# JaworWr/CUDA-ray-tracer

Hardware: AMD Instinct MI355X
Metric: Mrays/sec, 20spheres.yml @1920x1080 (higher is better)
Workload: dtype f64

## Files before the change

cuda-ray-tracer_amd/csrc/rt_capi.cpp:

```cpp
#include <hip/hip_runtime.h>

#include <algorithm>
#include <cmath>
#include <cstdarg>
#include <cstdio>
#include <cstdlib>
#include <cstring>
#include <memory>
#include <new>
#include <string>
#include <vector>

#include "mi355rt.h"
#include "rt_launch.h"
#include "rt_scene_dev.h"
#include "rt_scene_image.hpp"
#include "rt_frame_host.hpp"
#include "rt_set_scene.h"
#include "scene-exception.h"
#include "scene.h"
#include "camera.h"

#define RT_KERNELS(V)                                                                                                                              \
    {RT_CAT(rt_launch_trace, V), RT_CAT(rt_launch_wavefront, V),  RT_CAT(rt_launch_ray_list, V),      RT_CAT(rt_launch_gbuffer, V),   RT_CAT(rt_launch_pick, V), \
// ... 170 lines not shown
    bool zero_counters = false;
    DevMem<uint64_t> d_stamps;
    DevMem<double> d_camx, d_camy;
    size_t n_stamp_rows = 0;
    uint64_t frame = 0;
    uint32_t tag = 0;
    DevMem<uint32_t> d_order, d_tiles;
    MappedWords h_listed;
    uint32_t ord_split = 0;
    std::vector<double> cub_coefs;
    bool lean_ok = false;
    bool lean_now = true;
    uint32_t wg_slots = 1536;
    int lean_force = 0;
    bool ord_on = true;
    Staging pick;
    Staging ext;
    Staging rq;
    Scratch pth;
    DevMem<SetSceneStatus> d_ss_status;
    DevMem<unsigned char> d_ss_stage;
};

#ifdef RT_DIAGNOSTIC_BUILD
extern "C" int rt_abi_version(void) { return RT_ABI_VERSION | RT_ABI_DIAGNOSTIC; }
#else
extern "C" int rt_abi_version(void) { return RT_ABI_VERSION; }
#endif

extern "C" const char *rt_last_error(void) { return g_last_error.c_str(); }
// ... 222 lines not shown
    fa.height = rh;
    fa.max_refl = sd->max_reflections;
    fa.rank = cfg.rank;
    fa.world = cfg.world;
    fa.band_rows = kf * cfg.band_rows;
    fa.local_rows = kf * ctx->local_rows;
    fa.tiles_x = (rw + RT_TILE - 1) / RT_TILE;
    fa.n_tiles = fa.tiles_x * ((fa.local_rows + RT_TILE - 1) / RT_TILE);
    fa.rgba8 = (ctx->ssaa == 1u && cfg.format == RT_FMT_RGBA8) ? 1u : 0u;
    fa.ord_plain = (cfg.flags & RT_FLAG_PLAIN_ORDER) ? 1u : 0u;
    ctx->ord_split = (cfg.flags & RT_FLAG_NOSPLIT) ? 0u : RT_ORD_SPLIT_CLASSES;
    if (const char *e = std::getenv("MI355RT_SPLIT_CLASSES")) ctx->ord_split = (uint32_t) std::atoi(e) & 15u;
    int cus = 0;
    if (hipDeviceGetAttribute(&cus, hipDeviceAttributeMultiprocessorCount, device) == hipSuccess && cus > 0) ctx->wg_slots = 6u * (uint32_t) cus;
    if (const char *e = std::getenv("MI355RT_LEAN")) ctx->lean_force = (e[0] == 'a') ? 1 : ((e[0] == 'n') ? -1 : 0);
}

static int create_scene(rt_ctx *ctx, const rt_scene_desc *sd, rtp::SceneImage &im)
{
    FrameArgs &fa = ctx->fa;
    im = rtp::scene_image(*sd, ctx->cfg.flags, fa);
    ctx->cub_coefs = im.cub_coefs;
    ctx->lean_ok = im.lean_ok && !std::getenv("MI355RT_NOLEAN");
    if (!(ctx->cfg.flags & RT_FLAG_SIMPLE)) {
        const size_t lds = rt_wavefront_lds_bytes_strict(fa.stage_bytes, sd->n_lights, (int) fa.has_mirror, fa.cull ? fa.n_us : 0u, 0, fa.n_cub);
        if (lds > 160u * 1024u) return fail(RT_ERR_SCENE, "rt_create: scene needs %zu bytes of LDS per workgroup (limit 160 KiB)", lds);
    }
    if (ctx->adaptive && (size_t) sd->n_objects * (sizeof(DevObject) + sizeof(UsEntry)) > 160u * 1024u)
        return fail(RT_ERR_SCENE, "rt_create: adaptive supersampling stages %zu bytes of LDS per workgroup (limit 160 KiB)",
                    (size_t) sd->n_objects * (sizeof(DevObject) + sizeof(UsEntry)));
// ... 67 lines not shown
    return device_table(ctx->d_geo_xy, xy.data(), sizeof(uint32_t) * 2u * hpx, "halo coordinates");
}

static int create_order_state(rt_ctx *ctx)
{
    FrameArgs &fa = ctx->fa;
    const uint32_t flags = ctx->cfg.flags;
    if (!(flags & (RT_FLAG_SIMPLE | RT_FLAG_STATIC_ORDER)) && fa.n_tiles > 0 && fa.n_tiles <= RT_ORD_MAX_TILES) {
        fa.ord_stride = (RT_ORD_HDR + 17u * fa.n_tiles + 15u) & ~15u;
        if (int rc = device_table(ctx->d_order, nullptr, sizeof(uint32_t) * (3u * (size_t) fa.ord_stride + fa.n_tiles), "order")) return rc;
        fa.order_state = ctx->d_order;
        if (hipHostMalloc((void **) &ctx->h_listed.p, 64, hipHostMallocMapped | hipHostMallocPortable) == hipSuccess) {
            ctx->h_listed[0] = 0;
            ctx->h_listed[1] = 0;
            ctx->h_listed[2] = 0xFFFFFFFFu;
            if (hipHostGetDevicePointer((void **) &fa.ord_host, ctx->h_listed, 0) != hipSuccess) {
                ctx->h_listed.reset();
                fa.ord_host = nullptr;
            }
        } else {
            ctx->h_listed.p = nullptr;
            (void) hipGetLastError();
        }
    }
    if (!(flags & RT_FLAG_SIMPLE) && fa.all_cullable && fa.n_tiles > 0) {
        if (int rc = device_table(ctx->d_tiles, nullptr, sizeof(uint32_t) * fa.n_tiles, "tile state")) return rc;
        fa.tile_state = ctx->d_tiles;
    }
    ctx->zero_counters = std::getenv("MI355RT_DEBUG_COUNTERS") != nullptr;
    if (ctx->zero_counters) {
// ... 99 lines not shown
}

static int timer_end(rt_ctx *ctx, hipStream_t stream, float *ms)
{
    if (!ms) return RT_OK;
    RT_HIP(hipEventRecord(ctx->ev1, stream));
    RT_HIP(hipEventSynchronize(ctx->ev1));
    RT_HIP(hipEventElapsedTime(ms, ctx->ev0, ctx->ev1));
    return RT_OK;
}

static void choose_schedule(rt_ctx *ctx, FrameArgs &fa)
{
    if (ctx->lean_ok && ctx->h_listed && ctx->lean_force == 0) {
        const uint32_t tiles = ((volatile uint32_t *) ctx->h_listed.p)[2];
        if (ctx->lean_now ? (uint64_t) tiles * 100u < (uint64_t) ctx->wg_slots * 62u : (uint64_t) tiles * 100u >= (uint64_t) ctx->wg_slots * 66u) ctx->lean_now = !ctx->lean_now;
    } else {
        ctx->lean_now = ctx->lean_force >= 0;
    }
    static const bool debug_order = std::getenv("MI355RT_DEBUG_ORDER") != nullptr;
    if (debug_order && ctx->h_listed)
        std::fprintf(stderr, "mi355rt: frame %llu: tiles with hits %u, list slots wanted %u, census %u, schedule %s\n", (unsigned long long) ctx->frame, ((volatile uint32_t *) ctx->h_listed.p)[2],
                     ((volatile uint32_t *) ctx->h_listed.p)[0], ((volatile uint32_t *) ctx->h_listed.p)[1], ctx->lean_now ? "lean" : "general");
    fa.lean = (ctx->lean_ok && ctx->lean_now && !fa.sparse) ? 1u : 0u;
}

static int rotate_launch_order(rt_ctx *ctx, FrameArgs &fa, hipStream_t stream)
{
    fa.ord_read = (uint32_t) (ctx->frame % 3u);
    fa.ord_write = (uint32_t) ((ctx->frame + 1u) % 3u);
    fa.ord_zero = (uint32_t) ((ctx->frame + 2u) % 3u);
    uint32_t cap = fa.n_tiles;
    if (ctx->h_listed) {
        const uint32_t seen = ((volatile uint32_t *) ctx->h_listed.p)[0], census = ((volatile uint32_t *) ctx->h_listed.p)[1];
        const uint64_t want = (uint64_t) seen + seen / 4u + 64u;
        if (want < cap) cap = (uint32_t) want;
        const uint64_t with_hits = (uint64_t) census * 16u;
        const uint64_t slots = ctx->wg_slots ? ctx->wg_slots : 1536u;
        const bool too_many = ctx->ord_on ? with_hits * 3u >= slots * 16u : with_hits >= slots * 4u;
        const bool too_dense = ctx->ord_on ? with_hits * 4u >= fa.n_tiles : with_hits * 5u >= fa.n_tiles;
        ctx->ord_on = !(too_many || too_dense);
    }
    fa.ord_cap = cap;
    fa.ord_on = ctx->ord_on ? 1u : 0u;
    fa.ord_split = (fa.sparse || fa.lean) ? 0u : ctx->ord_split;
    fa.ord_frame = (uint32_t) (ctx->frame % 0xFFFFFFF0ull) + 1u;
    if (fa.ord_frame == 1u && ctx->frame != 0u)
        RT_HIP(hipMemsetAsync(fa.order_state + 3u * (size_t) fa.ord_stride, 0, sizeof(uint32_t) * fa.n_tiles, stream));
    ctx->frame++;
    return RT_OK;
}

static int render_impl(rt_ctx *ctx, const double cam[16], void *dev_fb, void *stream_, float *ms, bool sparse, uint32_t sparse_cap)
{
    hipStream_t stream = (hipStream_t) stream_;
    FrameArgs &fa = ctx->fa;
    const bool ss = ctx->ssaa > 1u && !ctx->adaptive;
// ... 450 lines not shown
    a.coefs = dev->coefs;
    a.reflection = dev->reflection;
    a.albedo = dev->albedo;
    a.light_p = dev->light_p;
    a.light_color = dev->light_color;
    a.n_obj = fa.n_obj;
    a.n_lights = fa.n_lights;
    a.n_us = fa.n_us;
    a.n_gq = fa.n_gq;
    a.n_lin = fa.n_lin;
    a.off_us = fa.off_us;
    a.off_gq = fa.off_gq;
    a.off_lin = fa.off_lin;
    a.off_mat = fa.off_mat;
    a.has_mirror = fa.has_mirror;
    const hipError_t e = rt_launch_set_scene(&a, stream);
    if (e != hipSuccess) return fail(RT_ERR_DEVICE, "%s: kernel launch failed: %s", who, hipGetErrorString(e));
    return order_end(ctx, stream, capturing);
}

extern "C" int rt_set_scene(rt_ctx *ctx, const rt_scene_update *dev, void *stream)
{
    if (!ctx || !dev) return fail(RT_ERR_INVALID, "rt_set_scene: null argument");
    if (int rc = set_scene_check("rt_set_scene", ctx, dev)) return rc;
    return set_scene_enqueue("rt_set_scene", ctx, dev, (hipStream_t) stream);
}

extern "C" int rt_set_scene_host(rt_ctx *ctx, const rt_scene_update *host, void *stream_)
{
    if (!ctx || !host) return fail(RT_ERR_INVALID, "rt_set_scene_host: null argument");
// ... 251 lines not shown
```

cuda-ray-tracer_amd/csrc/rt_frame_host.hpp:

```cpp
#ifndef RT_FRAME_HOST_HPP
#define RT_FRAME_HOST_HPP

#include <algorithm>
#include <cmath>
#include <cstring>
#include <vector>

#include "rt_math.hpp"
#include "rt_scene_dev.h"

namespace rtf {

inline void camera_tables(uint32_t nx, uint32_t ny, double aspect, double tan_half_fov, std::vector<double> &cx, std::vector<double> &cy)
{
    cx.resize(nx);
    cy.resize(ny);
    for (uint32_t x = 0; x < nx; x++) {
        const double ndc_x = ((int) x + 0.5) / (int) nx;
        cx[x] = (2.0 * ndc_x - 1.0) * aspect * tan_half_fov;
    }
    for (uint32_t y = 0; y < ny; y++) {
        const double ndc_y = ((int) y + 0.5) / (int) ny;
        cy[y] = (2.0 * ndc_y - 1.0) * tan_half_fov;
    }
// ... 30 lines not shown
    }
    fa.cx_a = 2.0 * fa.aspect * fa.tan_half_fov / (double) fa.width;
    fa.cx_b = (1.0 / (double) fa.width - 1.0) * fa.aspect * fa.tan_half_fov;
    fa.cy_a = 2.0 * fa.tan_half_fov / (double) fa.height;
    fa.cy_b = (1.0 / (double) fa.height - 1.0) * fa.tan_half_fov;
    if (!(fa.cx_a > 0.0) || !(fa.cy_a > 0.0) || !std::isfinite(fa.cx_a) || !std::isfinite(fa.cy_a)) fa.tile_planes_ok = 0;
}

inline int64_t halo_global_row(uint32_t h, uint32_t band_rows, uint32_t world, uint32_t rank, uint32_t local_rows)
{
    const uint32_t b = h >> 1, rows = std::min(band_rows, local_rows - b * band_rows);
    const int64_t g0 = ((int64_t) b * world + rank) * band_rows;
    return (h & 1u) ? g0 + rows : g0 - 1;
}

}

#endif
```

cuda-ray-tracer_amd/csrc/rt_scene_dev.h:

```cpp
#ifndef RT_SCENE_DEV_H
#define RT_SCENE_DEV_H

#include <stddef.h>
#include <stdint.h>

enum {
    K_X3 = 0, K_Y3, K_Z3, K_X2Y, K_XY2, K_X2Z, K_XZ2, K_Y2Z, K_YZ2, K_XYZ,
    K_X2, K_Y2, K_Z2, K_XY, K_XZ, K_YZ,
    K_X, K_Y, K_Z, K_C
};

#define RT_CLS_CUBIC 1u
#define RT_CLS_SQUARE 2u
#define RT_CLS_CROSS 4u
#define RT_CLS_UNITSQ 8u

struct alignas(16) DevObject {
    double c[20];
    float albedo[3];
    float refl;
    uint32_t cls;
    uint32_t pad[3];
    double bs_center[3];
    double bs_radius;
// ... 77 lines not shown
    uint32_t *ord_host;
    uint32_t ord_stride, ord_read, ord_write, ord_zero;
    uint32_t ord_cap;
    uint32_t ord_on;
    uint32_t ord_plain;
    uint32_t ord_frame;
    uint32_t ord_split;
    uint32_t *tile_state;
    uint32_t frame_tag;
    uint32_t n_scan;
    uint32_t lean;
    double cub_rec[4][10];
    double cub_abs[4][4];
    uint32_t lights_plain;
    uint32_t pt_mask[2];
};

#define RT_CUB_AT_MAX 4
#define RT_CUB_REC 10
static_assert(offsetof(FrameArgs, cub_abs) == offsetof(FrameArgs, cub_rec) + sizeof(double) * 4 * RT_CUB_REC, "cub_abs directly behind cub_rec");
#define RT_TILE 16
#define RT_SCAN_TILES 64
#define RT_PAINT_TILES 16
#define RT_ORD_SPLIT_CLASSES 8u
#define RT_ORD_HDR 32
#define RT_ORD_MAX_TILES 262144u

#endif
```

cuda-ray-tracer_amd/csrc/rt_wavefront.hip:

```cpp
#include <hip/hip_runtime.h>
#include <cstdlib>

#include "rt_launch.h"
#include "rt_math.hpp"
#include "rt_scene_dev.h"
#include "rt_wavefront_math.hpp"

#ifndef RT_VARIANT
#error "define RT_VARIANT=strict|fast"
#endif

namespace RT_SYM(rtw) {

using namespace rtm;

#define RT_LOAD_LIGHTK(lk, l) \
    LightK lk; \
    lk.p[0] = clight[l].p[0]; lk.p[1] = clight[l].p[1]; lk.p[2] = clight[l].p[2]; \
    lk.sdir[0] = clight[l].sdir[0]; lk.sdir[1] = clight[l].sdir[1]; lk.sdir[2] = clight[l].sdir[2]; \
    lk.u2 = clight[l].u2; lk.inv_uu = clight[l].inv_uu; lk.len_u = clight[l].len_u; lk.four_u2 = clight[l].four_u2; \
    lk.s_yz = clight[l].s_yz; lk.s_xz = clight[l].s_xz; lk.s_xy = clight[l].s_xy; \
    lk.color[0] = clight[l].color[0]; lk.color[1] = clight[l].color[1]; lk.color[2] = clight[l].color[2]; \
    lk.flags = clight[l].flags;
typedef const __attribute__((address_space(4))) LightK *ConstLights;
// ... 334 lines not shown
                for (uint32_t c = 0; c < ORD_CLASSES; c++) count = c == k ? oh.cnt[c] : count;
                if (pos < count && ord_last_position(oh, ord_first(oh, k) + pos) < n_eff && ord_rd[RT_ORD_HDR + (1u + k) * n_tiles + pos] == t) st = ST_COVERED;
            }
        }
        uint32_t expect = old;
        __hip_atomic_compare_exchange_strong(tile_state + t, &expect, (tag << ST_BITS) | st, __ATOMIC_RELAXED, __ATOMIC_RELAXED,
                                             __HIP_MEMORY_SCOPE_AGENT);
    }
    if (lane == 0) {
        const uint32_t first = blockIdx.x * RT_SCAN_TILES + wave * 16u;
        const uint32_t nt = first >= n_tiles ? 0u : (n_tiles - first < 16u ? n_tiles - first : 16u);
        cnt.cull(C_TILE, (unsigned long long) nt * n_us);
    }
}

__device__ __forceinline__ void paint_tiles(const FrameArgs &fa, uint32_t *tile_state, uint32_t tag, uint32_t n_tiles, void *fb, const F3 &bg, uint32_t block,
                                            uint32_t wave, uint32_t lane)
{
    const uint32_t sub = lane >> 4, j0 = lane & 15u;
    const uint32_t t = block * RT_PAINT_TILES + wave * 4u + sub;
    const bool tv = t < n_tiles;
    uint32_t v = (tag << ST_BITS) | ST_NONEMPTY;
    if (j0 == 0 && tv) v = tile_word_wait(tile_state + t, tag, tile_word_load(tile_state + t));
    const unsigned long long em = __ballot(j0 == 0 && tv && (v & ST_MASK) == ST_EMPTY);
    if (!((em >> (16u * sub)) & 1ull)) return;
    const uint32_t tile_x = t % fa.tiles_x, tile_y = t / fa.tiles_x;
    const uint32_t x = tile_x * RT_TILE + j0, y0l = tile_y * RT_TILE;
    if (x >= fa.width) return;
    if (fa.rgba8) {
        uchar4 px;
        px.x = (unsigned char) (int) (bg.x * 255.0f + 0.5f);
        px.y = (unsigned char) (int) (bg.y * 255.0f + 0.5f);
        px.z = (unsigned char) (int) (bg.z * 255.0f + 0.5f);
        px.w = 255;
        uchar4 *dst = reinterpret_cast<uchar4 *>(fb) + (size_t) y0l * fa.width + x;
#pragma unroll
        for (uint32_t row = 0; row < RT_TILE; row++)
            if (y0l + row < fa.local_rows) dst[(size_t) row * fa.width] = px;
    } else {
        const float4 px = make_float4(bg.x, bg.y, bg.z, 1.0f);
        float4 *dst = reinterpret_cast<float4 *>(fb) + (size_t) y0l * fa.width + x;
#pragma unroll
        for (uint32_t row = 0; row < RT_TILE; row++)
            if (y0l + row < fa.local_rows) dst[(size_t) row * fa.width] = px;
    }
}

template <bool COUNT, bool HAS_GQ, bool HAS_CUBIC, bool PRIMARY>
__device__ __forceinline__ void nearest(const FrameArgs &fa, const SceneLds &S, const DevObject *__restrict__ gobj, const Mono &m,
                                        bool live, uint32_t lane, double &best_t, int &best, Cnt<COUNT> &cnt)
{
    best = -1;
    best_t = INFINITY;
    const bool quad = fabs(m.u2) > EPS;
    const double four_t2 = 4.0 * m.u2;
    D3 axis{0.0, 0.0, 1.0};
    double cos_t = 1.0;
    const bool cone = PRIMARY && fa.cull;
    if (cone) {
        axis = D3{readlane_d(m.d.x, 36), readlane_d(m.d.y, 36), readlane_d(m.d.z, 36)};
// ... 295 lines not shown
    const unsigned char *hot_us;
    const uint32_t *hot_ord_rd;
    uint32_t hot_n_us, hot_ord_cap, hot_n_tiles, hot_flags;
    uint32_t *hot_tile_state;
    uint32_t hot_frame_tag, hot_n_scan;
};
struct ColdArgs {
    FrameArgs fa;
    const unsigned char *gscene;
    const DevLight *glight;
    void *fb;
    unsigned long long *counters;
    const double *camx, *camy;
};
static_assert(sizeof(HotArgs) == 48 && alignof(ColdArgs) == 8, "kernel argument layout");
__device__ __forceinline__ const ColdArgs &cold_args()
{
    typedef const __attribute__((address_space(4))) unsigned char *KernargBytes;
    KernargBytes p = (KernargBytes) __builtin_amdgcn_kernarg_segment_ptr();
    asm volatile("" : "+s"(p));
    return *(const ColdArgs *) (p + sizeof(HotArgs));
}

__device__ __forceinline__ bool lean_dir_blocked(const UsEntry *us, const CullRec *crec, const BoxH *boxp, const D3 &o, double u0, const LightK &lk, bool wanted,
                                                 uint32_t own, bool own_skip, unsigned long long own_excl, uint32_t n_us, uint32_t lane)
{
    const D3 d{lk.sdir[0], lk.sdir[1], lk.sdir[2]};
    unsigned long long it = __ballot(lane < n_us && crec_relevant(crec[lane], d, lk.inv_uu, lk.len_u));
    if (__popcll(it) >= BOX_STAGE_MIN) it &= __ballot(lane < n_us && crec_in_box_shadow(crec[lane], *boxp, d, lk.s_yz, lk.s_xz, lk.s_xy));
    it &= ~own_excl;
// ... 200 lines not shown
                        acc.x += col.x;
                        acc.y += col.y;
                        acc.z += col.z;
                    }
                }
                if (hit) {
                    res.x = (acc.x < 1.0f) ? acc.x : 1.0f;
                    res.y = (acc.y < 1.0f) ? acc.y : 1.0f;
                    res.z = (acc.z < 1.0f) ? acc.z : 1.0f;
                }
                if (listing_) b_ticks = __builtin_amdgcn_s_memtime() - b_t0;
                RT_STAMP(6);
            }
    }

template <bool COUNT, bool HAS_GQ, bool HAS_CUBIC, bool HAS_MIRROR, bool LEAN = false>
__global__ __launch_bounds__(256, (wf_occupancy<COUNT, HAS_GQ, HAS_CUBIC, HAS_MIRROR, LEAN>())) void wavefront_tile_kernel(
    const unsigned char *hot_us,
    const uint32_t *hot_ord_rd,
    uint32_t hot_n_us, uint32_t hot_ord_cap, uint32_t hot_n_tiles,
    uint32_t hot_flags,
    uint32_t *hot_tile_state,
    uint32_t hot_frame_tag, uint32_t hot_n_scan,
    const ColdArgs cold_never_named)
{
    const uint32_t tid = threadIdx.x, wave = (uint32_t) __builtin_amdgcn_readfirstlane((int) (threadIdx.x >> 6)), lane = tid & 63;
    constexpr bool ALL_SPHERES_POSSIBLE = !HAS_GQ && !HAS_CUBIC;
    const uint32_t ord_slots = (hot_flags & 2u) ? hot_ord_cap : 0u;
    uint32_t slot = blockIdx.x;
    uint32_t tstate = ST_TIMEOUT;
    uint32_t role = 0, paint_block = 0;
    if (ALL_SPHERES_POSSIBLE && hot_tile_state) {
        if (blockIdx.x < hot_n_scan) {
            role = 1;
        } else {
            slot -= hot_n_scan;
            if (slot >= ord_slots) {
                const uint32_t q = slot - ord_slots;
                if (hot_flags & 4u) {
                    const uint32_t grp = q / (RT_PAINT_TILES + 1u), pos = q - grp * (RT_PAINT_TILES + 1u);
                    if (pos == 0u) {
                        role = 2;
                        paint_block = grp;
                    }
                    slot = ord_slots + grp * RT_PAINT_TILES + (pos - 1u);
                    if (role == 0 && slot - ord_slots >= hot_n_tiles) return;
                }
                if (role == 0) {
                    uint32_t *w = hot_tile_state + (slot - ord_slots);
                    uint32_t v = 0;
                    if (lane == 0) v = tile_word_wait(w, hot_frame_tag, tile_word_load(w));
                    tstate = (uint32_t) __builtin_amdgcn_readfirstlane((int) v) & ST_MASK;
                    if (!COUNT && tstate == ST_EMPTY && slot != 0u) return;
                    if (tstate == ST_COVERED) return;
                }
            }
        }
    }
    const ColdArgs &cold = cold_args();
    const FrameArgs &fa = cold.fa;
    const unsigned char *__restrict__ gscene = cold.gscene;
    const DevLight *__restrict__ glight = cold.glight;
    void *__restrict__ fb = cold.fb;
    unsigned long long *__restrict__ counters = cold.counters;
    const double *__restrict__ camx = cold.camx, *__restrict__ camy = cold.camy;
    ConstLights clight = (ConstLights) (glight + fa.n_lights);
    constexpr bool OWNG = !HAS_GQ && !HAS_CUBIC;
    extern __shared__ __align__(16) unsigned char smem[];
    constexpr bool NEED_CROSS = HAS_GQ || HAS_CUBIC;
    static_assert(!LEAN || (!HAS_GQ && !HAS_CUBIC && !HAS_MIRROR), "the lean path renders unit spheres only");
    const LdsLayout L(fa.stage_bytes, fa.n_lights, HAS_MIRROR, fa.cull ? fa.n_us : 0u, LEAN, HAS_CUBIC ? fa.n_cub : 0u);
    const DevObject *gobj = reinterpret_cast<const DevObject *>(gscene);
    SceneLds S;
// ... 83 lines not shown
    if (hot_flags & 2u) {
        ord_wr = fa.order_state + (size_t) fa.ord_write * fa.ord_stride;
        asm volatile("" ::"s"(fa.cam[0]), "s"(fa.cam[2]), "s"(fa.cam[5]), "s"(fa.cam[6]), "s"(fa.cam[8]), "s"(fa.cam[10]), "s"(fa.origin[0]),
                     "s"(fa.origin[2]), "s"(fa.aspect), "s"(fa.tan_half_fov), "s"(fa.width), "s"(fa.local_rows), "s"(fa.tiles_x), "s"(fa.n_us),
                     "s"(fa.off_us), "s"(fa.band_rows), "s"(fa.all_cullable), "s"(gscene));
        if (wave == 0) {
            typedef const __attribute__((address_space(4))) uint32_t *ConstWords;
            ConstWords ord_rd = (ConstWords) hot_ord_rd;
            const OrdHeader oh = ord_header(ord_rd, ((hot_flags >> 4) & 15u) | ((hot_flags >> 20) << 4));
            const uint32_t idx_tile = slot >= ord_slots ? slot - ord_slots : 0u;
            const uint32_t w = ord_rd[RT_ORD_HDR + idx_tile];
            const uint32_t n_eff = ord_positions(oh) < hot_ord_cap ? ord_positions(oh) : hot_ord_cap;
            if (slot == 0 && lane == 0) {
                uint32_t *z = fa.order_state + (size_t) fa.ord_zero * fa.ord_stride;
                for (uint32_t k = 0; k < RT_ORD_HDR; k += 4) *reinterpret_cast<uint4 *>(z + k) = make_uint4(0, 0, 0, 0);
                if (fa.ord_host) { fa.ord_host[0] = oh.n_listed + oh.n_candidates; fa.ord_host[1] = oh.census; fa.ord_host[2] = oh.n_listed; }
            }
            uint32_t d_half = 0;
            uint32_t d_tile = slot, d_flags = oh.census * 64u < hot_n_tiles ? 4u : 0u;
            if (slot < ord_slots) {
                if (slot >= n_eff) {
                    d_flags |= 8u;
                } else {
                    const uint32_t p = (hot_flags & 8u) ? slot : ord_rank_of_slot(slot, n_eff, blockIdx.x - slot);
                    const uint32_t rank = p < 2u * oh.n_heavy ? p >> 1 : p - oh.n_heavy;
                    d_half = p < 2u * oh.n_heavy ? 1u + (p & 1u) : 0u;
                    uint32_t k, idx;
                    ord_locate(oh, rank, k, idx);
                    d_tile = ord_rd[RT_ORD_HDR + (1u + k) * hot_n_tiles + idx];
                    const uint32_t back = ord_rd[RT_ORD_HDR + (d_tile < hot_n_tiles ? d_tile : 0u)];
                    d_flags |= (d_tile >= hot_n_tiles || back != ((idx << 5) | (k + 1u)) || ord_last_position(oh, rank) >= n_eff) ? 8u : 1u;
// ... 479 lines not shown
            } else {
                reinterpret_cast<float4 *>(fb)[pix] = make_float4(res.x, res.y, res.z, 1.0f);
            }
        }
        if (ord_cls && ord_pos < fe.n_tiles) {
            ord_wr[RT_ORD_HDR + ord_cls * fe.n_tiles + ord_pos] = tile;
            ord_wr[RT_ORD_HDR + tile] = (ord_pos << 5) | ord_cls;
        }
        RT_STAMP(10);
    }

    RT_STAMP_FLUSH(counters, lane);
    cnt.flush(counters);
}


}

extern "C" size_t RT_SYM(rt_wavefront_lds_bytes)(uint32_t stage_bytes, uint32_t n_lights, int has_mirror, uint32_t n_cull_spheres, int lean, uint32_t n_cub)
{
    return RT_SYM(rtw)::LdsLayout(stage_bytes, n_lights, has_mirror != 0, n_cull_spheres, lean != 0, n_cub).total;
}

extern "C" hipError_t RT_SYM(rt_launch_wavefront)(const FrameArgs *fa, const DevObject *gobj, const DevLight *glight,
                                                   void *fb, unsigned long long *counters, int count,
                                                   const double *camx, const double *camy, hipStream_t stream)
{
    using namespace RT_SYM(rtw);
    if (fa->n_tiles == 0) return hipSuccess;
    const uint32_t n_scan = fa->tile_state ? fa->n_scan : 0u;
    const uint32_t n_paint = (n_scan && !fa->sparse) ? (fa->n_tiles + RT_PAINT_TILES - 1u) / RT_PAINT_TILES : 0u;
    const uint32_t n_index = n_paint ? n_paint * (RT_PAINT_TILES + 1u) : fa->n_tiles;
    const dim3 grid(n_scan + ((fa->order_state && fa->ord_on) ? fa->ord_cap : 0u) + n_index), block(WG);
    const unsigned char *gs = reinterpret_cast<const unsigned char *>(gobj);
    int sel = (count ? 8 : 0) | (fa->has_mirror ? 4 : 0) | (fa->n_gq ? 2 : 0) | (fa->n_cub ? 1 : 0);
    const bool lean = fa->lean && (sel & 7) == 0 && fa->all_cullable && fa->n_us == fa->n_obj && !fa->sparse;
    if (lean) sel = count ? 17 : 16;
    const size_t lds = LdsLayout(fa->stage_bytes, fa->n_lights, fa->has_mirror != 0, fa->cull ? fa->n_us : 0u, lean, fa->n_cub).total;
    const bool ordering = fa->order_state && fa->ord_on;
    const unsigned char *hot_us = gs + fa->off_us;
    const uint32_t *hot_ord_rd = ordering ? fa->order_state + (size_t) fa->ord_read * fa->ord_stride : nullptr;
    uint32_t hot_flags = (fa->all_cullable ? 1u : 0u) | (ordering ? 2u : 0u) | (n_paint ? 4u : 0u) | (fa->ord_plain ? 8u : 0u) |
                         ((fa->ord_split & 15u) << 4);
#ifdef RT_WF_DEBUG_EXITS
    if (const char *dbg = getenv("MI355RT_DEBUG_EXIT")) hot_flags |= (uint32_t) atoi(dbg) << 8;
#endif
    if (fa->ord_split && ordering) {
        struct SlotsKey { int dev, sel; size_t lds; uint32_t slots; };
        static thread_local SlotsKey memo[4] = {{-1, 0, 0, 0}, {-1, 0, 0, 0}, {-1, 0, 0, 0}, {-1, 0, 0, 0}};
        static thread_local unsigned memo_next = 0;
        int dev = 0;
        (void) hipGetDevice(&dev);
        uint32_t slots = 0;
        bool found = false;
        for (const SlotsKey &k : memo)
            if (k.dev == dev && k.sel == sel && k.lds == lds) { slots = k.slots; found = true; }
        if (!found) {
            int per_cu = 0, cus = 0;
#define RT_OCC(C, M, G, Q) (void) hipOccupancyMaxActiveBlocksPerMultiprocessor(&per_cu, wavefront_tile_kernel<C, G, Q, M>, WG, lds)
            switch (sel) {
            case 0: RT_OCC(false, false, false, false); break;
            case 1: RT_OCC(false, false, false, true); break;
            case 2: RT_OCC(false, false, true, false); break;
            case 3: RT_OCC(false, false, true, true); break;
            case 4: RT_OCC(false, true, false, false); break;
            case 5: RT_OCC(false, true, false, true); break;
            case 6: RT_OCC(false, true, true, false); break;
            case 7: RT_OCC(false, true, true, true); break;
            default: break;
            }
#undef RT_OCC
            (void) hipDeviceGetAttribute(&cus, hipDeviceAttributeMultiprocessorCount, dev);
            const long long total = (long long) (per_cu > 0 ? per_cu : 0) * (cus > 0 ? cus : 0);
            slots = (uint32_t) (total > 4095 ? 4095 : total);
            memo[memo_next++ & 3u] = SlotsKey{dev, sel, lds, slots};
        }
        hot_flags |= slots << 20;
    }
    const ColdArgs cold{*fa, gs, glight, fb, counters, camx, camy};
#define RT_LAUNCH(C, M, G, Q) hipLaunchKernelGGL((wavefront_tile_kernel<C, G, Q, M>), grid, block, lds, stream, hot_us, hot_ord_rd, fa->n_us, fa->ord_cap, fa->n_tiles, hot_flags, n_scan ? fa->tile_state : nullptr, fa->frame_tag, n_scan, cold)
    switch (sel) {
    case 0: RT_LAUNCH(false, false, false, false); break;
    case 1: RT_LAUNCH(false, false, false, true); break;
    case 2: RT_LAUNCH(false, false, true, false); break;
    case 3: RT_LAUNCH(false, false, true, true); break;
    case 4: RT_LAUNCH(false, true, false, false); break;
    case 5: RT_LAUNCH(false, true, false, true); break;
    case 6: RT_LAUNCH(false, true, true, false); break;
    case 7: RT_LAUNCH(false, true, true, true); break;
    case 8: RT_LAUNCH(true, false, false, false); break;
    case 9: RT_LAUNCH(true, false, false, true); break;
    case 10: RT_LAUNCH(true, false, true, false); break;
    case 11: RT_LAUNCH(true, false, true, true); break;
    case 12: RT_LAUNCH(true, true, false, false); break;
    case 13: RT_LAUNCH(true, true, false, true); break;
    case 14: RT_LAUNCH(true, true, true, false); break;
    case 15: RT_LAUNCH(true, true, true, true); break;
    case 16: hipLaunchKernelGGL((wavefront_tile_kernel<false, false, false, false, true>), grid, block, lds, stream, hot_us, hot_ord_rd, fa->n_us, fa->ord_cap, fa->n_tiles, hot_flags, n_scan ? fa->tile_state : nullptr, fa->frame_tag, n_scan, cold); break;
    default: hipLaunchKernelGGL((wavefront_tile_kernel<true, false, false, false, true>), grid, block, lds, stream, hot_us, hot_ord_rd, fa->n_us, fa->ord_cap, fa->n_tiles, hot_flags, n_scan ? fa->tile_state : nullptr, fa->frame_tag, n_scan, cold); break;
    }
#undef RT_LAUNCH
    return hipGetLastError();
}
```

Before: 205,000.

## Compact tile index grid into per-group workgroups that loop over non-empty tiles

```diff
diff --git a/cuda-ray-tracer_amd/csrc/rt_capi.cpp b/cuda-ray-tracer_amd/csrc/rt_capi.cpp
--- a/cuda-ray-tracer_amd/csrc/rt_capi.cpp
+++ b/cuda-ray-tracer_amd/csrc/rt_capi.cpp
@@ -208,6 +208,9 @@
     uint32_t wg_slots = 1536;
     int lean_force = 0;
     bool ord_on = true;
+    rtf::IndexRounds idx;
+    uint32_t idx_force = 0;
+    bool idx_event = false;
     Staging pick;
     Staging ext;
     Staging rq;
@@ -460,6 +463,9 @@
     int cus = 0;
     if (hipDeviceGetAttribute(&cus, hipDeviceAttributeMultiprocessorCount, device) == hipSuccess && cus > 0) ctx->wg_slots = 6u * (uint32_t) cus;
     if (const char *e = std::getenv("MI355RT_LEAN")) ctx->lean_force = (e[0] == 'a') ? 1 : ((e[0] == 'n') ? -1 : 0);
+    fa.idx_plain = std::getenv("MI355RT_INDEX_SLOTS") ? 1u : 0u;
+    fa.idx_rounds = RT_IDX_ROUNDS_MAX;
+    if (const char *e = std::getenv("MI355RT_INDEX_ROUNDS")) ctx->idx_force = (uint32_t) std::atoi(e);
 }
 
 static int create_scene(rt_ctx *ctx, const rt_scene_desc *sd, rtp::SceneImage &im)
@@ -557,6 +563,7 @@
             ctx->h_listed[0] = 0;
             ctx->h_listed[1] = 0;
             ctx->h_listed[2] = 0xFFFFFFFFu;
+            ctx->h_listed[3] = 0;
             if (hipHostGetDevicePointer((void **) &fa.ord_host, ctx->h_listed, 0) != hipSuccess) {
                 ctx->h_listed.reset();
                 fa.ord_host = nullptr;
@@ -686,7 +693,10 @@
 {
     if (ctx->lean_ok && ctx->h_listed && ctx->lean_force == 0) {
         const uint32_t tiles = ((volatile uint32_t *) ctx->h_listed.p)[2];
-        if (ctx->lean_now ? (uint64_t) tiles * 100u < (uint64_t) ctx->wg_slots * 62u : (uint64_t) tiles * 100u >= (uint64_t) ctx->wg_slots * 66u) ctx->lean_now = !ctx->lean_now;
+        if (ctx->lean_now ? (uint64_t) tiles * 100u < (uint64_t) ctx->wg_slots * 62u : (uint64_t) tiles * 100u >= (uint64_t) ctx->wg_slots * 66u) {
+            ctx->lean_now = !ctx->lean_now;
+            ctx->idx_event = true;
+        }
     } else {
         ctx->lean_now = ctx->lean_force >= 0;
     }
@@ -711,8 +721,14 @@
         const uint64_t slots = ctx->wg_slots ? ctx->wg_slots : 1536u;
         const bool too_many = ctx->ord_on ? with_hits * 3u >= slots * 16u : with_hits >= slots * 4u;
         const bool too_dense = ctx->ord_on ? with_hits * 4u >= fa.n_tiles : with_hits * 5u >= fa.n_tiles;
+        if (ctx->ord_on == (too_many || too_dense)) ctx->idx_event = true;
         ctx->ord_on = !(too_many || too_dense);
-    }
+        fa.idx_rounds = rtf::choose_index_rounds(ctx->idx, ctx->idx_event, census, ((volatile uint32_t *) ctx->h_listed.p)[2], ((volatile uint32_t *) ctx->h_listed.p)[3]);
+        ctx->idx_event = false;
+    } else {
+        fa.idx_rounds = RT_IDX_ROUNDS_MAX;
+    }
+    if (ctx->idx_force >= 1u && ctx->idx_force <= RT_IDX_ROUNDS_MAX) fa.idx_rounds = ctx->idx_force;
     fa.ord_cap = cap;
     fa.ord_on = ctx->ord_on ? 1u : 0u;
     fa.ord_split = (fa.sparse || fa.lean) ? 0u : ctx->ord_split;
@@ -1193,6 +1209,7 @@
     a.off_lin = fa.off_lin;
     a.off_mat = fa.off_mat;
     a.has_mirror = fa.has_mirror;
+    ctx->idx_event = true;
     const hipError_t e = rt_launch_set_scene(&a, stream);
     if (e != hipSuccess) return fail(RT_ERR_DEVICE, "%s: kernel launch failed: %s", who, hipGetErrorString(e));
     return order_end(ctx, stream, capturing);
diff --git a/cuda-ray-tracer_amd/csrc/rt_frame_host.hpp b/cuda-ray-tracer_amd/csrc/rt_frame_host.hpp
--- a/cuda-ray-tracer_amd/csrc/rt_frame_host.hpp
+++ b/cuda-ray-tracer_amd/csrc/rt_frame_host.hpp
@@ -68,6 +68,26 @@
     return (h & 1u) ? g0 + rows : g0 - 1;
 }
 
+constexpr uint32_t RT_IDX_HOLD = 8u;
+struct IndexRounds {
+    uint32_t hold = RT_IDX_HOLD;
+    uint32_t census = 0xFFFFFFFFu, listed = 0xFFFFFFFFu;
+};
+inline uint32_t choose_index_rounds(IndexRounds &st, bool event, uint32_t census, uint32_t listed, uint32_t left)
+{
+    if (event) st.hold = RT_IDX_HOLD;
+    if (census != st.census || listed != st.listed) {
+        st.hold = std::max(st.hold, 2u);
+        st.census = census;
+        st.listed = listed;
+    }
+    if (st.hold) {
+        st.hold--;
+        return RT_IDX_ROUNDS_MAX;
+    }
+    return 1u << rt_index_rounds_log2(std::max(left, 1u));
+}
+
 }
 
 #endif
diff --git a/cuda-ray-tracer_amd/csrc/rt_scene_dev.h b/cuda-ray-tracer_amd/csrc/rt_scene_dev.h
--- a/cuda-ray-tracer_amd/csrc/rt_scene_dev.h
+++ b/cuda-ray-tracer_amd/csrc/rt_scene_dev.h
@@ -115,6 +115,8 @@
     double cub_abs[4][4];
     uint32_t lights_plain;
     uint32_t pt_mask[2];
+    uint32_t idx_rounds;
+    uint32_t idx_plain;
 };
 
 #define RT_CUB_AT_MAX 4
@@ -125,6 +127,28 @@
 #define RT_PAINT_TILES 16
 #define RT_ORD_SPLIT_CLASSES 8u
 #define RT_ORD_HDR 32
+#define RT_ORD_LEFT 18
+#define RT_IDX_ROUNDS_MAX 16u
 #define RT_ORD_MAX_TILES 262144u
 
+
+static inline uint32_t rt_index_rounds_log2(uint32_t idx_rounds)
+{
+    const uint32_t r = (idx_rounds == 0u || idx_rounds > RT_IDX_ROUNDS_MAX) ? RT_IDX_ROUNDS_MAX : idx_rounds;
+    uint32_t lg = 0;
+    while ((1u << lg) < r) lg++;
+    return lg;
+}
+static inline uint32_t rt_index_region(uint32_t n_tiles, bool paint, bool groups, uint32_t lg_rounds)
+{
+    const uint32_t n_groups = (n_tiles + RT_PAINT_TILES - 1u) / RT_PAINT_TILES;
+    if (groups) return n_groups << lg_rounds;
+    return paint ? n_groups * (RT_PAINT_TILES + 1u) : n_tiles;
+}
+
+static inline uint32_t rt_wavefront_grid(uint32_t n_scan, uint32_t ord_slots, uint32_t n_tiles, bool paint, bool groups, uint32_t lg_rounds)
+{
+    return n_scan + ord_slots + rt_index_region(n_tiles, paint, groups, lg_rounds);
+}
+
 #endif
diff --git a/cuda-ray-tracer_amd/csrc/rt_wavefront.hip b/cuda-ray-tracer_amd/csrc/rt_wavefront.hip
--- a/cuda-ray-tracer_amd/csrc/rt_wavefront.hip
+++ b/cuda-ray-tracer_amd/csrc/rt_wavefront.hip
@@ -372,16 +372,8 @@
     }
 }
 
-__device__ __forceinline__ void paint_tiles(const FrameArgs &fa, uint32_t *tile_state, uint32_t tag, uint32_t n_tiles, void *fb, const F3 &bg, uint32_t block,
-                                            uint32_t wave, uint32_t lane)
-{
-    const uint32_t sub = lane >> 4, j0 = lane & 15u;
-    const uint32_t t = block * RT_PAINT_TILES + wave * 4u + sub;
-    const bool tv = t < n_tiles;
-    uint32_t v = (tag << ST_BITS) | ST_NONEMPTY;
-    if (j0 == 0 && tv) v = tile_word_wait(tile_state + t, tag, tile_word_load(tile_state + t));
-    const unsigned long long em = __ballot(j0 == 0 && tv && (v & ST_MASK) == ST_EMPTY);
-    if (!((em >> (16u * sub)) & 1ull)) return;
+__device__ __forceinline__ void paint_tile_column(const FrameArgs &fa, void *fb, const F3 &bg, uint32_t t, uint32_t j0)
+{
     const uint32_t tile_x = t % fa.tiles_x, tile_y = t / fa.tiles_x;
     const uint32_t x = tile_x * RT_TILE + j0, y0l = tile_y * RT_TILE;
     if (x >= fa.width) return;
@@ -402,6 +394,25 @@
         for (uint32_t row = 0; row < RT_TILE; row++)
             if (y0l + row < fa.local_rows) dst[(size_t) row * fa.width] = px;
     }
+}
+
+__device__ __forceinline__ void paint_tiles(const FrameArgs &fa, uint32_t *tile_state, uint32_t tag, uint32_t n_tiles, void *fb, const F3 &bg, uint32_t block,
+                                            uint32_t wave, uint32_t lane)
+{
+    const uint32_t sub = lane >> 4, j0 = lane & 15u;
+    const uint32_t t = block * RT_PAINT_TILES + wave * 4u + sub;
+    const bool tv = t < n_tiles;
+    uint32_t v = (tag << ST_BITS) | ST_NONEMPTY;
+    if (j0 == 0 && tv) v = tile_word_wait(tile_state + t, tag, tile_word_load(tile_state + t));
+    const unsigned long long em = __ballot(j0 == 0 && tv && (v & ST_MASK) == ST_EMPTY);
+    if (!((em >> (16u * sub)) & 1ull)) return;
+    paint_tile_column(fa, fb, bg, t, j0);
+}
+
+__device__ __forceinline__ void paint_group(const FrameArgs &fa, void *fb, const F3 &bg, uint32_t block, uint32_t empty, uint32_t wave, uint32_t lane)
+{
+    const uint32_t sub = lane >> 4, j0 = lane & 15u, i = wave * 4u + sub;
+    if ((empty >> i) & 1u) paint_tile_column(fa, fb, bg, block * RT_PAINT_TILES + i, j0);
 }
 
 template <bool COUNT, bool HAS_GQ, bool HAS_CUBIC, bool PRIMARY>
@@ -727,6 +738,13 @@
     const double *camx, *camy;
 };
 static_assert(sizeof(HotArgs) == 48 && alignof(ColdArgs) == 8, "kernel argument layout");
+__device__ __forceinline__ const HotArgs &hot_args()
+{
+    typedef const __attribute__((address_space(4))) unsigned char *KernargBytes;
+    KernargBytes p = (KernargBytes) __builtin_amdgcn_kernarg_segment_ptr();
+    asm volatile("" : "+s"(p));
+    return *(const HotArgs *) p;
+}
 __device__ __forceinline__ const ColdArgs &cold_args()
 {
     typedef const __attribute__((address_space(4))) unsigned char *KernargBytes;
@@ -957,49 +975,16 @@
             }
     }
 
-template <bool COUNT, bool HAS_GQ, bool HAS_CUBIC, bool HAS_MIRROR, bool LEAN = false>
-__global__ __launch_bounds__(256, (wf_occupancy<COUNT, HAS_GQ, HAS_CUBIC, HAS_MIRROR, LEAN>())) void wavefront_tile_kernel(
-    const unsigned char *hot_us,
-    const uint32_t *hot_ord_rd,
-    uint32_t hot_n_us, uint32_t hot_ord_cap, uint32_t hot_n_tiles,
-    uint32_t hot_flags,
-    uint32_t *hot_tile_state,
-    uint32_t hot_frame_tag, uint32_t hot_n_scan,
-    const ColdArgs cold_never_named)
-{
-    const uint32_t tid = threadIdx.x, wave = (uint32_t) __builtin_amdgcn_readfirstlane((int) (threadIdx.x >> 6)), lane = tid & 63;
+template <bool COUNT, bool HAS_GQ, bool HAS_CUBIC, bool HAS_MIRROR, bool LEAN>
+__device__ __forceinline__ void wavefront_tile_body(const unsigned char *hot_us, const uint32_t *hot_ord_rd, uint32_t hot_n_us, uint32_t hot_ord_cap, uint32_t hot_n_tiles,
+                                                    uint32_t hot_flags, uint32_t *hot_tile_state, uint32_t hot_frame_tag, uint32_t slot, uint32_t tstate, uint32_t role,
+                                                    uint32_t paint_block)
+{
     constexpr bool ALL_SPHERES_POSSIBLE = !HAS_GQ && !HAS_CUBIC;
+    uint32_t tid0_ = threadIdx.x;
+    if constexpr (ALL_SPHERES_POSSIBLE && !COUNT) asm volatile("" : "+v"(tid0_));
+    const uint32_t tid = tid0_, wave = (uint32_t) __builtin_amdgcn_readfirstlane((int) (tid >> 6)), lane = tid & 63;
     const uint32_t ord_slots = (hot_flags & 2u) ? hot_ord_cap : 0u;
-    uint32_t slot = blockIdx.x;
-    uint32_t tstate = ST_TIMEOUT;
-    uint32_t role = 0, paint_block = 0;
-    if (ALL_SPHERES_POSSIBLE && hot_tile_state) {
-        if (blockIdx.x < hot_n_scan) {
-            role = 1;
-        } else {
-            slot -= hot_n_scan;
-            if (slot >= ord_slots) {
-                const uint32_t q = slot - ord_slots;
-                if (hot_flags & 4u) {
-                    const uint32_t grp = q / (RT_PAINT_TILES + 1u), pos = q - grp * (RT_PAINT_TILES + 1u);
-                    if (pos == 0u) {
-                        role = 2;
-                        paint_block = grp;
-                    }
-                    slot = ord_slots + grp * RT_PAINT_TILES + (pos - 1u);
-                    if (role == 0 && slot - ord_slots >= hot_n_tiles) return;
-                }
-                if (role == 0) {
-                    uint32_t *w = hot_tile_state + (slot - ord_slots);
-                    uint32_t v = 0;
-                    if (lane == 0) v = tile_word_wait(w, hot_frame_tag, tile_word_load(w));
-                    tstate = (uint32_t) __builtin_amdgcn_readfirstlane((int) v) & ST_MASK;
-                    if (!COUNT && tstate == ST_EMPTY && slot != 0u) return;
-                    if (tstate == ST_COVERED) return;
-                }
-            }
-        }
-    }
     const ColdArgs &cold = cold_args();
     const FrameArgs &fa = cold.fa;
     const unsigned char *__restrict__ gscene = cold.gscene;
@@ -1113,7 +1098,7 @@
             if (slot == 0 && lane == 0) {
                 uint32_t *z = fa.order_state + (size_t) fa.ord_zero * fa.ord_stride;
                 for (uint32_t k = 0; k < RT_ORD_HDR; k += 4) *reinterpret_cast<uint4 *>(z + k) = make_uint4(0, 0, 0, 0);
-                if (fa.ord_host) { fa.ord_host[0] = oh.n_listed + oh.n_candidates; fa.ord_host[1] = oh.census; fa.ord_host[2] = oh.n_listed; }
+                if (fa.ord_host) { fa.ord_host[0] = oh.n_listed + oh.n_candidates; fa.ord_host[1] = oh.census; fa.ord_host[2] = oh.n_listed; fa.ord_host[3] = ord_rd[RT_ORD_LEFT]; }
             }
             uint32_t d_half = 0;
             uint32_t d_tile = slot, d_flags = oh.census * 64u < hot_n_tiles ? 4u : 0u;
@@ -1623,8 +1608,133 @@
     cnt.flush(counters);
 }
 
-
-}
+template <bool COUNT, bool HAS_GQ, bool HAS_CUBIC, bool HAS_MIRROR, bool LEAN = false>
+__global__ __launch_bounds__(256, (wf_occupancy<COUNT, HAS_GQ, HAS_CUBIC, HAS_MIRROR, LEAN>())) void wavefront_tile_kernel(
+    const unsigned char *hot_us,
+    const uint32_t *hot_ord_rd,
+    uint32_t hot_n_us, uint32_t hot_ord_cap, uint32_t hot_n_tiles,
+    uint32_t hot_flags,
+    uint32_t *hot_tile_state,
+    uint32_t hot_frame_tag, uint32_t hot_n_scan,
+    const ColdArgs cold_never_named)
+{
+    const uint32_t wave = (uint32_t) __builtin_amdgcn_readfirstlane((int) (threadIdx.x >> 6)), lane = threadIdx.x & 63;
+    constexpr bool ALL_SPHERES_POSSIBLE = !HAS_GQ && !HAS_CUBIC;
+    constexpr bool GROUPS = ALL_SPHERES_POSSIBLE && !COUNT;
+    const uint32_t ord_slots = (hot_flags & 2u) ? hot_ord_cap : 0u;
+    uint32_t slot = blockIdx.x;
+    uint32_t tstate = ST_TIMEOUT;
+    uint32_t role = 0, paint_block = 0;
+    uint32_t rest = 0;
+    if (ALL_SPHERES_POSSIBLE && hot_tile_state) {
+        if (blockIdx.x < hot_n_scan) {
+            role = 1;
+        } else {
+            slot -= hot_n_scan;
+            if (slot >= ord_slots) {
+                const uint32_t q = slot - ord_slots;
+                if (GROUPS && (hot_flags & 0x806u) == 0x6u) {
+                    const uint32_t lg = (hot_flags >> 12) & 7u, round = q & ((1u << lg) - 1u), grp = q >> lg;
+                    const uint32_t t = grp * RT_PAINT_TILES + (lane & 15u);
+                    const bool tv = lane < RT_PAINT_TILES && t < hot_n_tiles;
+                    uint32_t v = 0;
+                    if (tv) v = tile_word_wait(hot_tile_state + t, hot_frame_tag, tile_word_load(hot_tile_state + t));
+                    const uint32_t st = v & ST_MASK;
+                    const uint32_t empty = (uint32_t) __ballot(tv && st == ST_EMPTY);
+                    const uint32_t timeout = (uint32_t) __ballot(tv && st == ST_TIMEOUT);
+                    rest = (uint32_t) __ballot(tv && st == ST_NONEMPTY) | timeout;
+                    if (round == 0u && (empty | rest) != 0u) {
+                        const ColdArgs &cold = cold_args();
+                        if (empty) paint_group(cold.fa, cold.fb, F3{cold.fa.bg[0], cold.fa.bg[1], cold.fa.bg[2]}, grp, empty, wave, lane);
+                        if (rest != 0u && threadIdx.x == 0) atomicMax(cold.fa.order_state + (size_t) cold.fa.ord_write * cold.fa.ord_stride + RT_ORD_LEFT, (uint32_t) __popc(rest));
+                    }
+                    for (uint32_t i = 0; i < round; i++) rest &= rest - 1u;
+                    if (rest == 0u) return;
+                    if (round + 1u < (1u << lg)) rest &= 0u - rest;
+                    const uint32_t i = (uint32_t) __builtin_ctz(rest);
+                    rest &= rest - 1u;
+                    slot = ord_slots + grp * RT_PAINT_TILES + i;
+                    tstate = ((timeout >> i) & 1u) ? ST_TIMEOUT : ST_NONEMPTY;
+                } else {
+                    if (hot_flags & 4u) {
+                        const uint32_t grp = q / (RT_PAINT_TILES + 1u), pos = q - grp * (RT_PAINT_TILES + 1u);
+                        if (pos == 0u) {
+                            role = 2;
+                            paint_block = grp;
+                        }
+                        slot = ord_slots + grp * RT_PAINT_TILES + (pos - 1u);
+                        if (role == 0 && slot - ord_slots >= hot_n_tiles) return;
+                    }
+                    if (role == 0) {
+                        uint32_t *w = hot_tile_state + (slot - ord_slots);
+                        uint32_t v = 0;
+                        if (lane == 0) v = tile_word_wait(w, hot_frame_tag, tile_word_load(w));
+                        tstate = (uint32_t) __builtin_amdgcn_readfirstlane((int) v) & ST_MASK;
+                        if (!COUNT && tstate == ST_EMPTY && slot != 0u) return;
+                        if (tstate == ST_COVERED) return;
+                    }
+                }
+            }
+        }
+    }
+    if constexpr (!GROUPS) {
+        wavefront_tile_body<COUNT, HAS_GQ, HAS_CUBIC, HAS_MIRROR, LEAN>(hot_us, hot_ord_rd, hot_n_us, hot_ord_cap, hot_n_tiles, hot_flags, hot_tile_state, hot_frame_tag, slot,
+                                                                        tstate, role, paint_block);
+        return;
+    }
+    for (;;) {
+        wavefront_tile_body<COUNT, HAS_GQ, HAS_CUBIC, HAS_MIRROR, LEAN>(hot_us, hot_ord_rd, hot_n_us, hot_ord_cap, hot_n_tiles, hot_flags, hot_tile_state, hot_frame_tag, slot,
+                                                                        tstate, role, paint_block);
+        if (rest == 0u) return;
+        lds_barrier();
+        const HotArgs &hot = hot_args();
+        hot_us = hot.hot_us; hot_ord_rd = hot.hot_ord_rd; hot_n_us = hot.hot_n_us; hot_ord_cap = hot.hot_ord_cap; hot_n_tiles = hot.hot_n_tiles;
+        hot_flags = hot.hot_flags; hot_tile_state = hot.hot_tile_state; hot_frame_tag = hot.hot_frame_tag;
+        const uint32_t i = (uint32_t) __builtin_ctz(rest);
+        rest &= rest - 1u;
+        const uint32_t slot0 = (hot_flags & 2u) ? hot_ord_cap : 0u, t = ((blockIdx.x - hot.hot_n_scan - slot0) >> ((hot_flags >> 12) & 7u)) * RT_PAINT_TILES + i;
+        slot = slot0 + t;
+        tstate = (uint32_t) __builtin_amdgcn_readfirstlane((int) tile_word_load(hot_tile_state + t)) & ST_MASK;
+    }
+}
+
+}
+
+#ifndef RT_WF_PART
+#define RT_WF_PART 2
+#endif
+#define RT_WF_LAUNCH_ARGS hot_us, hot_ord_rd, n_us, ord_cap, n_tiles, hot_flags, tile_state, frame_tag, n_scan, *cold
+#if RT_WF_PART != 0
+extern "C" hipError_t RT_SYM(rt_launch_wavefront_groups)(int sel, uint32_t grid_x, size_t lds, hipStream_t stream, const unsigned char *hot_us, const uint32_t *hot_ord_rd,
+                                                          uint32_t n_us, uint32_t ord_cap, uint32_t n_tiles, uint32_t hot_flags, uint32_t *tile_state, uint32_t frame_tag,
+                                                          uint32_t n_scan, const void *cold_)
+{
+    using namespace RT_SYM(rtw);
+    const ColdArgs *cold = static_cast<const ColdArgs *>(cold_);
+    const dim3 grid(grid_x), block(WG);
+    switch (sel) {
+    case 0: hipLaunchKernelGGL((wavefront_tile_kernel<false, false, false, false>), grid, block, lds, stream, RT_WF_LAUNCH_ARGS); break;
+    case 4: hipLaunchKernelGGL((wavefront_tile_kernel<false, false, false, true>), grid, block, lds, stream, RT_WF_LAUNCH_ARGS); break;
+    case 16: hipLaunchKernelGGL((wavefront_tile_kernel<false, false, false, false, true>), grid, block, lds, stream, RT_WF_LAUNCH_ARGS); break;
+    default: return hipErrorInvalidValue;
+    }
+    return hipGetLastError();
+}
+extern "C" int RT_SYM(rt_wavefront_groups_per_cu)(int sel, size_t lds)
+{
+    using namespace RT_SYM(rtw);
+    int per_cu = 0;
+    if (sel == 0) (void) hipOccupancyMaxActiveBlocksPerMultiprocessor(&per_cu, wavefront_tile_kernel<false, false, false, false>, WG, lds);
+    if (sel == 4) (void) hipOccupancyMaxActiveBlocksPerMultiprocessor(&per_cu, wavefront_tile_kernel<false, false, false, true>, WG, lds);
+    return per_cu;
+}
+#else
+extern "C" hipError_t RT_SYM(rt_launch_wavefront_groups)(int sel, uint32_t grid_x, size_t lds, hipStream_t stream, const unsigned char *hot_us, const uint32_t *hot_ord_rd,
+                                                          uint32_t n_us, uint32_t ord_cap, uint32_t n_tiles, uint32_t hot_flags, uint32_t *tile_state, uint32_t frame_tag,
+                                                          uint32_t n_scan, const void *cold_);
+extern "C" int RT_SYM(rt_wavefront_groups_per_cu)(int sel, size_t lds);
+#endif
+#if RT_WF_PART != 1
 
 extern "C" size_t RT_SYM(rt_wavefront_lds_bytes)(uint32_t stage_bytes, uint32_t n_lights, int has_mirror, uint32_t n_cull_spheres, int lean, uint32_t n_cub)
 {
@@ -1639,18 +1749,20 @@
     if (fa->n_tiles == 0) return hipSuccess;
     const uint32_t n_scan = fa->tile_state ? fa->n_scan : 0u;
     const uint32_t n_paint = (n_scan && !fa->sparse) ? (fa->n_tiles + RT_PAINT_TILES - 1u) / RT_PAINT_TILES : 0u;
-    const uint32_t n_index = n_paint ? n_paint * (RT_PAINT_TILES + 1u) : fa->n_tiles;
-    const dim3 grid(n_scan + ((fa->order_state && fa->ord_on) ? fa->ord_cap : 0u) + n_index), block(WG);
+    const bool ordering = fa->order_state && fa->ord_on;
+    const uint32_t lg_rounds = rt_index_rounds_log2(fa->idx_rounds);
+    const bool groups = n_paint && ordering && !count && !fa->idx_plain && fa->n_gq == 0u && fa->n_cub == 0u;
+    const dim3 grid(rt_wavefront_grid(n_scan, ordering ? fa->ord_cap : 0u, fa->n_tiles, n_paint != 0u, groups, lg_rounds)), block(WG);
     const unsigned char *gs = reinterpret_cast<const unsigned char *>(gobj);
     int sel = (count ? 8 : 0) | (fa->has_mirror ? 4 : 0) | (fa->n_gq ? 2 : 0) | (fa->n_cub ? 1 : 0);
     const bool lean = fa->lean && (sel & 7) == 0 && fa->all_cullable && fa->n_us == fa->n_obj && !fa->sparse;
     if (lean) sel = count ? 17 : 16;
     const size_t lds = LdsLayout(fa->stage_bytes, fa->n_lights, fa->has_mirror != 0, fa->cull ? fa->n_us : 0u, lean, fa->n_cub).total;
-    const bool ordering = fa->order_state && fa->ord_on;
     const unsigned char *hot_us = gs + fa->off_us;
     const uint32_t *hot_ord_rd = ordering ? fa->order_state + (size_t) fa->ord_read * fa->ord_stride : nullptr;
     uint32_t hot_flags = (fa->all_cullable ? 1u : 0u) | (ordering ? 2u : 0u) | (n_paint ? 4u : 0u) | (fa->ord_plain ? 8u : 0u) |
-                         ((fa->ord_split & 15u) << 4);
+                         ((fa->ord_split & 15u) << 4) |
+                         (groups ? lg_rounds << 12 : 0x800u);
 #ifdef RT_WF_DEBUG_EXITS
     if (const char *dbg = getenv("MI355RT_DEBUG_EXIT")) hot_flags |= (uint32_t) atoi(dbg) << 8;
 #endif
@@ -1668,11 +1780,11 @@
             int per_cu = 0, cus = 0;
 #define RT_OCC(C, M, G, Q) (void) hipOccupancyMaxActiveBlocksPerMultiprocessor(&per_cu, wavefront_tile_kernel<C, G, Q, M>, WG, lds)
             switch (sel) {
-            case 0: RT_OCC(false, false, false, false); break;
+            case 0: per_cu = RT_SYM(rt_wavefront_groups_per_cu)(sel, lds); break;
             case 1: RT_OCC(false, false, false, true); break;
             case 2: RT_OCC(false, false, true, false); break;
             case 3: RT_OCC(false, false, true, true); break;
-            case 4: RT_OCC(false, true, false, false); break;
+            case 4: per_cu = RT_SYM(rt_wavefront_groups_per_cu)(sel, lds); break;
             case 5: RT_OCC(false, true, false, true); break;
             case 6: RT_OCC(false, true, true, false); break;
             case 7: RT_OCC(false, true, true, true); break;
@@ -1689,11 +1801,12 @@
     const ColdArgs cold{*fa, gs, glight, fb, counters, camx, camy};
 #define RT_LAUNCH(C, M, G, Q) hipLaunchKernelGGL((wavefront_tile_kernel<C, G, Q, M>), grid, block, lds, stream, hot_us, hot_ord_rd, fa->n_us, fa->ord_cap, fa->n_tiles, hot_flags, n_scan ? fa->tile_state : nullptr, fa->frame_tag, n_scan, cold)
     switch (sel) {
-    case 0: RT_LAUNCH(false, false, false, false); break;
+    case 0: case 4: case 16:
+        return RT_SYM(rt_launch_wavefront_groups)(sel, grid.x, lds, stream, hot_us, hot_ord_rd, fa->n_us, fa->ord_cap, fa->n_tiles, hot_flags, n_scan ? fa->tile_state : nullptr,
+                                                  fa->frame_tag, n_scan, &cold);
     case 1: RT_LAUNCH(false, false, false, true); break;
     case 2: RT_LAUNCH(false, false, true, false); break;
     case 3: RT_LAUNCH(false, false, true, true); break;
-    case 4: RT_LAUNCH(false, true, false, false); break;
     case 5: RT_LAUNCH(false, true, false, true); break;
     case 6: RT_LAUNCH(false, true, true, false); break;
     case 7: RT_LAUNCH(false, true, true, true); break;
@@ -1705,9 +1818,9 @@
     case 13: RT_LAUNCH(true, true, false, true); break;
     case 14: RT_LAUNCH(true, true, true, false); break;
     case 15: RT_LAUNCH(true, true, true, true); break;
-    case 16: hipLaunchKernelGGL((wavefront_tile_kernel<false, false, false, false, true>), grid, block, lds, stream, hot_us, hot_ord_rd, fa->n_us, fa->ord_cap, fa->n_tiles, hot_flags, n_scan ? fa->tile_state : nullptr, fa->frame_tag, n_scan, cold); break;
     default: hipLaunchKernelGGL((wavefront_tile_kernel<true, false, false, false, true>), grid, block, lds, stream, hot_us, hot_ord_rd, fa->n_us, fa->ord_cap, fa->n_tiles, hot_flags, n_scan ? fa->tile_state : nullptr, fa->frame_tag, n_scan, cold); break;
     }
 #undef RT_LAUNCH
     return hipGetLastError();
 }
+#endif
```

After: 140,600. -31.4%, worse.
